# JettHuang/jet-pbrt

Hardware: AMD Instinct MI355X
Metric: Msamples/sec (whole node) + per-pixel L2 vs CPU ref, cornell_box 1024spp (higher is better)
Workload: dtype f32

## Files before the change

### jet-pbrt_amd/csrc/jp_common.h

```cpp
#pragma once
#include "jp_shading.h"

using namespace jp;

extern __shared__ float4 s_dyn[];

#define JP_SHADE_CLASSES 6

struct DevCounters
{
	unsigned int n_queue[2];
	unsigned int n_shadow;
	unsigned int pad;
	unsigned long long closest, closest_hit, shadow, shadow_occ;
	unsigned long long cert_fallback;
};

struct Queues
{
	float4 *ray_o[2], *ray_d[2], *beta[2];
	float2 *hit;
	float4 *lacc;
	float4 *sh_o;
	float4 *sh_d, *sh_c;
	unsigned int *blk_q[2], *blk_sh;
	unsigned int cap;
	unsigned int R;
};

struct RenderConst
{
	int width, height, spp, max_depth;
	unsigned int seed;
	int band_rows, shard_index, shard_count;
	int npix;
	int local_rows;
	int s0, sbatch;
	int n_planes;
	int tiled;
	int compact;
	int slot_bits;
	int sampler_debug;
	int class_mask;
	int lane_index, lane_count, lane_rows;
};

__device__ __forceinline__ float rngf(const RenderConst& rc, uint32_t key, uint32_t dim) { return rc.sampler_debug ? 0.5f : jp_rng_float(key, dim); }

#define FLAG_BOUNCE(f) ((f) & 0xff)
#define FLAG_SPEC(f)   (((f) >> 8) & 1)
#define FLAG_DIM(f)    (((unsigned)(f)) >> 16)
#define MK_FLAGS(bounce, spec, dim) (((bounce) & 0xff) | ((spec) ? 0x100 : 0) | ((int)(dim) << 16))

__device__ __forceinline__ void pixel_of(const RenderConst& rc, int pix, int& x, int& y)
{
	int lx, r;
	if (rc.tiled)
	{
		const int t = pix >> 6, i = pix & 63, tpr = rc.width >> 4;
		const int ty = t / tpr, tx = t - ty * tpr;
		lx = (tx << 4) + (i & 15); r = (ty << 2) + (i >> 4);
	}
	else { r = pix / rc.width; lx = pix - r * rc.width; }
	x = lx;
	if (rc.lane_count > 1) { const int m = r / rc.lane_rows; r = (rc.lane_index + m * rc.lane_count) * rc.lane_rows + (r - m * rc.lane_rows); }
	const int j = r / rc.band_rows;
	y = (rc.shard_index + j * rc.shard_count) * rc.band_rows + (r - j * rc.band_rows);
}

__device__ __forceinline__ unsigned int wave_take(unsigned int* ctr, unsigned int n)
{
	unsigned int v = 0;
	if ((threadIdx.x & 63) == 0) v = atomicAdd(ctr, n);
	return (unsigned int)__builtin_amdgcn_readfirstlane((int)v);
}


#define JP_TEX_IMAGE_TAG 0x80000000u
#define JP_TEX_COLOR_TAG 0x40000000u
struct TexView
{
	const int4* desc;
	const float4* col;
	const unsigned int* texels;
	const int* mat_tex;
	const float2* prim_uv;
	unsigned int* side;
};
```

### jet-pbrt_amd/csrc/jp_kernels.hip

```cpp
#include "jp_common.h"
#include "jp_tex.h"
#include "jp_xbsdf.h"

#include <cstdio>
#include <cstring>
#include <string>
#include <vector>
#include <algorithm>
#include <cmath>
#include <mutex>
#include <thread>
#include "jp_lbvh.h"
#include "jp_ploc.h"

__global__ void __launch_bounds__(JP_BLOCK) k_raygen(SceneView sc, Queues q, RenderConst rc, DevCounters* cnt)
{
	const unsigned int total = (unsigned int)rc.npix * rc.sbatch;
	const unsigned int nchunks = (total + JP_BLOCK - 1) / JP_BLOCK;
	const unsigned int G = gridDim.x, b = blockIdx.x;
	if (b == 0 && threadIdx.x == 0) { cnt->n_queue[0] = total; cnt->n_queue[1] = 0; cnt->n_shadow = 0; }
	unsigned int filled = 0;
	const unsigned int K = (nchunks + G - 1) / G, npb = (unsigned int)rc.npix / JP_BLOCK;
	for (unsigned int k = 0, j0 = 0; k < K; k++, j0 += JP_BLOCK)
	{
// ... 51 lines not shown
template <> struct SceneAccess<1>
{
	float4 *nodes, *prims; int* stack; int depth;
	__device__ __forceinline__ SceneAccess(const SceneView& sc, int depth_) : depth(depth_)
	{
		stack = (int*)s_dyn + threadIdx.x;
		nodes = s_dyn + (depth * JP_BLOCK) / 4;
		prims = nodes + 5 * sc.n_nodes;
		for (int i = threadIdx.x; i < 4 * sc.n_nodes; i += JP_BLOCK) nodes[5 * (i >> 2) + (i & 3)] = sc.nodes[i];
		for (int i = threadIdx.x; i < 4 * sc.n_prims; i += JP_BLOCK) prims[5 * (i >> 2) + (i & 3)] = sc.prims[i];
		__syncthreads();
	}
	template <bool kAnyHit> __device__ __forceinline__ int trace(const SceneView&, V3 o, V3 d, float tmin, float& tmax) const
	{ return traverse<kAnyHit, 5>(nodes, prims, o, d, tmin, tmax, stack); }
};
template <> struct SceneAccess<2>
{
	float4* prims;
	__device__ __forceinline__ SceneAccess(const SceneView& sc, int)
	{
		prims = s_dyn;
		for (int i = threadIdx.x; i < 4 * sc.n_prims; i += JP_BLOCK) prims[5 * (i >> 2) + (i & 3)] = sc.prims[i];
		__syncthreads();
	}
	template <bool kAnyHit> __device__ __forceinline__ int trace(const SceneView& sc, V3 o, V3 d, float tmin, float& tmax) const
	{ return traverse_flat<kAnyHit, 5>(sc.flat, sc.n_flat, sc.n_prims, prims, o, d, tmin, tmax); }
};

template <> struct SceneAccess<3>
{
	const float4* prims; unsigned int* stack;
	__device__ __forceinline__ SceneAccess(const SceneView& sc, int) : prims(sc.prims), stack((unsigned int*)s_dyn + threadIdx.x) {}
	template <bool kAnyHit> __device__ __forceinline__ int trace(const SceneView& sc, V3 o, V3 d, float tmin, float& tmax) const
	{ return traverse_wide<kAnyHit>(sc.wide, prims, o, d, tmin, tmax, stack); }
};

template <> struct SceneAccess<4>
{
	WalkStack stack;
	__device__ __forceinline__ SceneAccess(const SceneView&, int depth) { stack.lds = (int*)s_dyn + threadIdx.x; stack.spill = nullptr; stack.cap = depth - 1; stack.stride = 0; }
	template <bool kAnyHit> __device__ __forceinline__ int trace(const SceneView& sc, V3 o, V3 d, float tmin, float& tmax) const
	{ return walk_ray<4, kAnyHit>(sc, o, d, tmin, tmax, stack); }
};

template <> struct SceneAccess<6>
{
	WalkStack stack;
	__device__ __forceinline__ SceneAccess(const SceneView&, int depth) { stack.lds = (int*)s_dyn + threadIdx.x; stack.spill = nullptr; stack.cap = depth - 1; stack.stride = 0; }
	template <bool kAnyHit> __device__ __forceinline__ int trace(const SceneView& sc, V3 o, V3 d, float tmin, float& tmax) const
	{ return walk_ray<6, kAnyHit>(sc, o, d, tmin, tmax, stack); }
};

template <> struct SceneAccess<5>
{
	const float4 *nodes, *prims; int* stack;
	__device__ __forceinline__ SceneAccess(const SceneView& sc, int) : nodes(sc.nodes), prims(sc.prims), stack((int*)s_dyn + threadIdx.x) {}
	template <bool kAnyHit> __device__ __forceinline__ int trace(const SceneView&, V3 o, V3 d, float tmin, float& tmax) const
	{ return traverse_ref<kAnyHit>(nodes, prims, o, d, tmin, tmax, stack); }
};

template <int kMode>
__global__ void __launch_bounds__(JP_BLOCK) k_extend(SceneView sc, Queues q, int cur, int depth, DevCounters* cnt)
{
	SceneAccess<kMode> acc(sc, depth);
	const unsigned int b = blockIdx.x, n = q.blk_q[cur][b], rbase = b * q.R;
	if (b == 0 && threadIdx.x == 0) { cnt->closest += cnt->n_queue[cur]; cnt->n_queue[cur ^ 1] = 0; cnt->n_shadow = 0; }
	unsigned int h = 0;
	float4 ro = make_float4(0, 0, 0, 0), rd = make_float4(0, 0, 1, 0);
	if (threadIdx.x < n) { ro = q.ray_o[cur][rbase + threadIdx.x]; rd = q.ray_d[cur][rbase + threadIdx.x]; }
	for (unsigned int j = threadIdx.x; j < n; j += JP_BLOCK)
	{
		const unsigned int i = rbase + j;
		const float4 co = ro, cd = rd;
		if (j + JP_BLOCK < n) { ro = q.ray_o[cur][i + JP_BLOCK]; rd = q.ray_d[cur][i + JP_BLOCK]; }
		float tmax = JP_INF;
		const int hit = acc.template trace<false>(sc, xyz(co), xyz(cd), 0.001f, tmax);
		q.hit[i] = make_float2(tmax, __int_as_float(hit));
		h += hit >= 0 ? 1u : 0u;
	}
	for (int off = 32; off > 0; off >>= 1) h += __shfl_down(h, off);
	if ((threadIdx.x & 63) == 0 && h) atomicAdd(&cnt->closest_hit, (unsigned long long)h);
}

#ifndef JP_SHADE_TILE
#define JP_SHADE_TILE 8192
#endif
template <bool kTab, bool kPrims, bool kStage, bool kSort, bool kTex>
__device__ __forceinline__ void shade_body(SceneView sc, Queues q, RenderConst rc, int cur, DevCounters* cnt, const TexView& tv)
{
	static_assert(kTab || !kPrims, "k_shade: primitive records in LDS only together with the tables");
	constexpr int kWaves = JP_BLOCK / 64, kMaxSeg = (JP_SHADE_TILE / JP_BLOCK) * kWaves;
	static_assert(JP_SHADE_TILE % JP_BLOCK == 0 && JP_SHADE_TILE <= 65536, "k_shade: tile positions are 16-bit");
	__shared__ unsigned short s_idx[kSort ? JP_SHADE_TILE : 1];
	__shared__ unsigned char s_key[kSort ? JP_SHADE_TILE : 1];
	__shared__ unsigned int s_cnt[kSort ? JP_SHADE_CLASSES * kMaxSeg : 1];
	__shared__ unsigned int s_wsum[kWaves];
	__shared__ unsigned int s_ctr[3];
	const unsigned int lane = threadIdx.x & 63u;
	const int n_tab = 2 * sc.n_lights + 4 * sc.n_mats + (sc.n_mats + 3) / 4, n_tab_all = n_tab + (kPrims ? 8 * sc.n_prims : 0);
	float4* s_lights = s_dyn;
	float4* s_mats = s_lights + 2 * sc.n_lights;
	int* s_mtype = (int*)(s_mats + 4 * sc.n_mats);
	float4* s_prims = s_dyn + n_tab;
	int4* s_meta = (int4*)(s_prims + 4 * sc.n_prims);
	const float4* s_frames = s_prims + 5 * sc.n_prims;
	float4* s_stage = s_dyn + n_tab_all + threadIdx.x;
	const unsigned int b = blockIdx.x, n = q.blk_q[cur][b];
	const int nxt = cur ^ 1;
#ifdef JP_SHADE_TIMING
	unsigned long long t_acc[10] = { 0, 0, 0, 0, 0, 0, 0, 0, 0, 0 }, t_last = __builtin_amdgcn_s_memtime();
#endif
	if (kTab)
	{
		for (int i = threadIdx.x; i < n_tab_all; i += 2 * JP_BLOCK)
		{
			const bool two = i + JP_BLOCK < n_tab_all;
			const float4 a = sc.shade_tab[i], c2 = two ? sc.shade_tab[i + JP_BLOCK] : a;
			s_dyn[i] = a; if (two) s_dyn[i + JP_BLOCK] = c2;
		}
	}
	if (n == 0) { if (threadIdx.x == 0) { q.blk_q[nxt][b] = 0; q.blk_sh[b] = 0; } return; }
	if (threadIdx.x == 0) { s_ctr[0] = 0; s_ctr[1] = 0; s_ctr[2] = 0; }
	__syncthreads();
	const float4* lights = kTab ? (const float4*)s_lights : sc.lights;
	const float4* mats = kTab ? (const float4*)s_mats : sc.mats;
	const int* mat_type = kTab ? (const int*)s_mtype : sc.mat_type;
	const float4* prims = kPrims ? (const float4*)s_prims : sc.prims;
	const int4* meta_t = kPrims ? (const int4*)s_meta : sc.meta;
	const unsigned int rbase = b * q.R;
	const unsigned int t0 = 0, count = n;
	JP_TS(0);
	if (kSort)
	{
		constexpr unsigned int seg = kMaxSeg, nctr = JP_SHADE_CLASSES * kMaxSeg;
		const unsigned int tid = threadIdx.x;
		const unsigned int plane = tid & 63u, wave = tid >> 6, npass = (count + JP_BLOCK - 1) / JP_BLOCK;
		const unsigned long long ltm = (1ull << plane) - 1ull;
		#pragma unroll 1
		for (unsigned int r0 = 0; r0 < npass; r0 += 8)
		{
			int pi[8];
			#pragma unroll
			for (int u = 0; u < 8; u++)
			{
				const unsigned int j = (r0 + u) * JP_BLOCK + tid;
				pi[u] = j < count ? __float_as_int(q.hit[rbase + t0 + j].y) : -2;
			}
			#pragma unroll
			for (int u = 0; u < 8; u++)
			{
				const unsigned int r = r0 + u;
				if (r >= npass) break;
				unsigned int key = JP_SHADE_CLASSES;
				if (pi[u] != -2)
				{
					int m = -1; if (pi[u] >= 0) m = meta_t[pi[u]].y;
					key = m >= 0 ? 1u + (unsigned int)mat_type[m] : 0u;
				}
				s_key[r * JP_BLOCK + tid] = (unsigned char)key;
				unsigned int mine = 0;
				#pragma unroll
				for (int c = 0; c < JP_SHADE_CLASSES; c++)
				{
					unsigned int nc = 0;
					if ((rc.class_mask >> c) & 1) nc = (unsigned int)__popcll(__ballot(key == (unsigned int)c));
					if (plane == (unsigned int)c) mine = nc;
				}
				if (plane < JP_SHADE_CLASSES) s_cnt[plane * seg + r * kWaves + wave] = mine;
			}
		}
		__syncthreads();
		{
			static_assert(JP_SHADE_CLASSES * kMaxSeg <= 3 * JP_BLOCK, "k_shade: three counters per thread");
			unsigned int v[3], t = 0;
			#pragma unroll
			for (int i = 0; i < 3; i++)
			{
				const unsigned int at = 3 * tid + i;
				v[i] = (at < nctr && (at % seg) / kWaves < npass) ? s_cnt[at] : 0u; t += v[i];
			}
			unsigned int incl = t;
			#pragma unroll
			for (int off = 1; off < 64; off <<= 1) { const unsigned int o = __shfl_up(incl, off); if (plane >= (unsigned int)off) incl += o; }
			if (plane == 63) s_wsum[wave] = incl;
			__syncthreads();
			unsigned int base = incl - t;
			#pragma unroll
			for (int w = 0; w < kWaves; w++) if ((unsigned int)w < wave) base += s_wsum[w];
			#pragma unroll
// ... 174 lines not shown
		JP_TS(5);
#ifdef JP_DBG_SKIP_SAMPLE
		if (false)
#else
		if (shaded)
#endif
		{
			const float ux = rngf(rc, key, dim), uy = rngf(rc, key, dim + 1); dim += 2;
			BsdfSample bs = sample_local(c, wo, ux, uy);
			bs.wi = to_world(fr, bs.wi);
			if (!(isblack(bs.f) || bs.pdf == 0.f))
			{
				nspec = (bs.flags & BS_SPECULAR) != 0;
				if (bounce >= 3)
				{
					const float qq = smax(0.05f, 1 - maxcomp(bs.f));
					const float ur = rngf(rc, key, dim++);
					if (!(ur < qq))
					{
						nbeta = cmul(beta, bs.f * absdot(bs.wi, N) / (bs.pdf * (1 - qq)));
						alive = true;
					}
				}
				else
				{
					nbeta = cmul(beta, bs.f * absdot(bs.wi, N) / bs.pdf);
					alive = true;
				}
				nd = bs.wi; nbounce = bounce + 1;
			}
		}
		JP_TS(6);
		unsigned int j = 0;
		const unsigned long long lt = (1ull << lane) - 1ull;
		const unsigned long long ma = __ballot(alive);
		if (kStage)
		{
			const unsigned long long ms = __ballot(k > 0);
			if (ma | ms)
			{
				const unsigned int base = wave_take(&s_ctr[1], (unsigned int)__popcll(ma) | ((unsigned int)__popcll(ms) << 16));
				j = rbase + (base & 0xffffu) + (unsigned int)__popcll(ma & lt);
				qs = rbase + (base >> 16) + (unsigned int)__popcll(ms & lt);
			}
			if (k > 0)
			{
				q.sh_o[qs] = make_float4(p.x, p.y, p.z, __int_as_float(slot | (k << rc.slot_bits)));
				for (int kk = 0; kk < k; kk++)
				{
					q.sh_d[(size_t)kk * q.cap + qs] = s_stage[(2 * kk) * JP_BLOCK];
					q.sh_c[(size_t)kk * q.cap + qs] = s_stage[(2 * kk + 1) * JP_BLOCK];
				}
			}
		}
		else if (ma) j = rbase + wave_take(&s_ctr[1], (unsigned int)__popcll(ma)) + (unsigned int)__popcll(ma & lt);
		if (alive)
		{
			q.ray_o[nxt][j] = make_float4(p.x, p.y, p.z, __int_as_float(slot));
			q.ray_d[nxt][j] = make_float4(nd.x, nd.y, nd.z, __int_as_float(MK_FLAGS(nbounce, nspec, dim)));
			q.beta[nxt][j] = make_float4(nbeta.x, nbeta.y, nbeta.z, __int_as_float((int)key));
		}
		JP_TS(7);
#ifdef JP_SHADE_TIMING
		asm volatile("s_waitcnt vmcnt(0)" ::: "memory");
		JP_TS(9);
#endif
	}
	JP_TS(2);
	__syncthreads();
	JP_TS(8);
#ifdef JP_SHADE_TIMING
	if (lane == 0) for (int i = 0; i < 10; i++) atomicAdd(&g_shade_t[i], t_acc[i]);
	if (lane == 0) atomicAdd(&g_shade_t[15], 1ull);
#endif
	if (threadIdx.x == 0)
	{
		const unsigned int run_q = kStage ? (s_ctr[1] & 0xffffu) : s_ctr[1], run_sh = kStage ? (s_ctr[1] >> 16) : s_ctr[2];
		q.blk_q[nxt][b] = run_q; q.blk_sh[b] = run_sh;
		if (run_q) atomicAdd(&cnt->n_queue[nxt], run_q);
		if (run_sh) atomicAdd(&cnt->n_shadow, run_sh);
	}
}
template <bool kTab, bool kPrims, bool kStage, bool kSort>
__global__ void __launch_bounds__(JP_BLOCK) k_shade(SceneView sc, Queues q, RenderConst rc, int cur, DevCounters* cnt)
{
	const TexView tv = {};
	shade_body<kTab, kPrims, kStage, kSort, false>(sc, q, rc, cur, cnt, tv);
}

template <int kMode>
__global__ void __launch_bounds__(JP_BLOCK, 4) k_shadow(SceneView sc, Queues q, RenderConst rc, int depth, DevCounters* cnt)
{
#ifdef JP_TRAV_TIMING
	unsigned long long t_acc[10] = { 0, 0, 0, 0, 0, 0, 0, 0, 0, 0 }, t_last = __builtin_amdgcn_s_memtime();
#endif
	SceneAccess<kMode> acc(sc, depth);
	const unsigned int b = blockIdx.x, E = q.blk_sh[b], rbase = b * q.R;
	JP_TT(0);
	unsigned int rays = 0, occ = 0;
	float4 so_n = make_float4(0, 0, 0, 0), sd_n = make_float4(0, 0, 1, 0);
	if (threadIdx.x < E) { so_n = q.sh_o[rbase + threadIdx.x]; sd_n = q.sh_d[rbase + threadIdx.x]; }
	for (unsigned int j = threadIdx.x; j < E; j += JP_BLOCK)
	{
		const unsigned int e = rbase + j;
#ifdef JP_TRAV_TIMING
		JP_TT(1);
		asm volatile("s_waitcnt vmcnt(0)" ::: "memory");
		JP_TT(2);
#endif
		const float4 so = so_n; float4 sd = sd_n;
		if (j + JP_BLOCK < E) { so_n = q.sh_o[e + JP_BLOCK]; sd_n = q.sh_d[e + JP_BLOCK]; }
		const int packed = __float_as_int(so.w);
		const int slot = packed & ((1 << rc.slot_bits) - 1), n = (int)((unsigned int)packed >> rc.slot_bits);
		if (n == 0) continue;
		bool any = false;
		const float4 L = q.lacc[slot];
		V3 a = mk(L.x, L.y, L.z);
		for (int k = 0; k < n; k++)
		{
			const float4 c4 = q.sh_c[(size_t)k * q.cap + e];
			float tmax = sd.w;
			const V3 dir = xyz(sd);
			if (k + 1 < n) sd = q.sh_d[(size_t)(k + 1) * q.cap + e];
			JP_TT(3);
#ifdef JP_TRAV_TIMING
			int hit;
			if constexpr (kMode == 2)
			{
				const unsigned int m = flat_boxes<false>(sc.flat, sc.n_flat, xyz(so), dir, 0.001f, tmax);
				JP_TT(4);
				hit = flat_prims<true, false, 5>(m, acc.prims, xyz(so), dir, 0.001f, tmax);
				JP_TT(5);
			}
			else hit = acc.template trace<true>(sc, xyz(so), dir, 0.001f, tmax);
#else
			const int hit = acc.template trace<true>(sc, xyz(so), dir, 0.001f, tmax);
#endif
			rays++;
			if (hit >= 0) occ++;
			else { a = a + xyz(c4); any = true; }
			JP_TT(6);
		}
		if (any) q.lacc[slot] = make_float4(a.x, a.y, a.z, 0.f);
		JP_TT(7);
	}
#ifdef JP_TRAV_TIMING
	JP_TT(1);
	if ((threadIdx.x & 63) == 0) { for (int i = 0; i < 8; i++) atomicAdd(&g_shade_t[i], t_acc[i]); atomicAdd(&g_shade_t[15], 1ull); }
#endif
	for (int off = 32; off > 0; off >>= 1) { rays += __shfl_down(rays, off); occ += __shfl_down(occ, off); }
	if ((threadIdx.x & 63) == 0) { if (rays) atomicAdd(&cnt->shadow, (unsigned long long)rays); if (occ) atomicAdd(&cnt->shadow_occ, (unsigned long long)occ); }
}

template <int kMode, bool kAnyHit, bool kVote>
__device__ __forceinline__ void persist_turn(Walker<kMode>& w, const SceneView& sc, const WalkStack& stack, bool pool)
{
	const int nh = __popcll(__ballot(!w.done && w.heavy())), nl = __popcll(__ballot(!w.done && !w.heavy()));
	const bool heavyTurn = kVote ? nh > nl : w.heavy();
	if (kVote) { JP_TURN(heavyTurn ? 3 : 0, 1); JP_TURN(heavyTurn ? 4 : 1, heavyTurn ? nh : nl); JP_TURN(heavyTurn ? 5 : 2, nh + nl); if (!pool) { JP_TURN(8, 1); JP_TURN(9, nh + nl); JP_TURN(10, heavyTurn ? nh : nl); } }
	if (!w.done && (w.heavy() == heavyTurn)) w.template step<kAnyHit>(sc, stack);
}
__device__ __forceinline__ unsigned int lane_rank(unsigned long long m) { return __builtin_amdgcn_mbcnt_hi((unsigned int)(m >> 32), __builtin_amdgcn_mbcnt_lo((unsigned int)m, 0u)); }

#ifndef JP_CERT_WAVES
#define JP_CERT_WAVES 8
#endif
template <int kMode, int kRefill, bool kVote>
// ... 451 lines not shown
```

### jet-pbrt_amd/csrc/jp_shading.h

```cpp
#pragma once
#include "jp_device.h"
#define JP_HD_INLINE __host__ __device__ __forceinline__

namespace jp
{
__device__ __forceinline__ void sincos_d(float xf, double* s, double* c)
{
	const double x = (double)xf;
	const double kd = rint(x * 0.63661977236758134308);
	const int k = (int)kd;
	double r = fma(-kd, 1.57079632679489655800e+00, x);
	r = fma(-kd, 6.12323399573676603587e-17, r);
	const double r2 = r * r;
	double sp = fma(r2, -7.6471637318198164759e-13, 1.6059043836821614599e-10);
	sp = fma(sp, r2, -2.5052108385441718775e-08);
	sp = fma(sp, r2, 2.7557319223985890653e-06);
	sp = fma(sp, r2, -1.9841269841269841270e-04);
	sp = fma(sp, r2, 8.3333333333333333333e-03);
	sp = fma(sp, r2, -1.6666666666666666667e-01);
	sp = fma(sp * r2, r, r);
	double cp = fma(r2, 4.7794773323873852974e-14, -1.1470745597729724714e-11);
	cp = fma(cp, r2, 2.0876756987868098979e-09);
	cp = fma(cp, r2, -2.7557319223985890653e-07);
	cp = fma(cp, r2, 2.4801587301587301587e-05);
	cp = fma(cp, r2, -1.3888888888888888889e-03);
	cp = fma(cp, r2, 4.1666666666666666667e-02);
	cp = fma(cp, r2, -0.5);
	cp = fma(cp, r2, 1.0);
	const double ss = (k & 1) ? cp : sp, cc = (k & 1) ? sp : cp;
	*s = (k & 2) ? -ss : ss;
	*c = ((k + 1) & 2) ? -cc : cc;
}

__device__ __constant__ int g_sincosf_mode = 0;

template <bool kFma>
JP_HD_INLINE void sincosf_libm(float y, float* sp, float* cp)
{
	union { float f; unsigned int u; } bits; bits.f = y;
	const unsigned int top = (bits.u >> 20) & 0x7ffu;
	const double x = (double)y;
	double xs, x2; int n = 0;
	if (top <= 0x3f3u)
	{
		if (top <= 0x397u) { *sp = y; *cp = 1.0f; return; }
		xs = x; x2 = x * x;
	}
	else
	{
		const double r = x * 0x1.45f306dc9c883p+23;
		n = ((int)r + 0x800000) >> 24;
		const double xr = kFma ? fma(-(double)n, 0x1.921fb54442d18p+0, x) : x - (double)n * 0x1.921fb54442d18p+0;
		const double sgn = ((n & 3) == 1 || (n & 3) == 2) ? -1.0 : 1.0;
		xs = xr * sgn; x2 = xr * xr;
	}
	const double t = (n & 2) ? -1.0 : 1.0;
	const double c0 = t, c1 = t * -0x1.ffffffd0c621cp-2, c2 = t * 0x1.55553e1068f19p-5, c3 = t * -0x1.6c087e89a359dp-10, c4 = t * 0x1.99343027bf8c3p-16;
	const double s1 = -0x1.555545995a603p-3, s2 = 0x1.1107605230bc4p-7, s3 = -0x1.994eb3774cf24p-13;
	const double x3 = x2 * xs, x4 = x2 * x2;
	const double x5 = x2 * x3, x6 = x2 * x4;
	double c1v, as, ac, bs, bc, S, C;
	if (kFma)
	{
		c1v = fma(x2, c1, c0); as = fma(x2, s3, s2); ac = fma(x2, c4, c3);
		bs = fma(x3, s1, xs); bc = fma(x4, c2, c1v);
		S = fma(as, x5, bs); C = fma(ac, x6, bc);
	}
	else
	{
		c1v = c0 + x2 * c1; as = s2 + x2 * s3; ac = c3 + x2 * c4;
		bs = xs + x3 * s1; bc = c1v + x4 * c2;
		S = bs + x5 * as; C = bc + x6 * ac;
	}
	const float fs = (float)S, fc = (float)C;
	if (n & 1) { *sp = fc; *cp = fs; } else { *sp = fs; *cp = fc; }
}

__device__ __forceinline__ void sincos_f(float xf, float* s, float* c)
{
	const int mode = g_sincosf_mode;
	if (mode == 1 && fabsf(xf) < 120.f) sincosf_libm<true>(xf, s, c);
	else if (mode == 2 && fabsf(xf) < 120.f) sincosf_libm<false>(xf, s, c);
	else { double sd, cd; sincos_d(xf, &sd, &cd); *s = (float)sd; *c = (float)cd; }
}

#define JP_2PI      (2.0f * JP_PI)
#define JP_PI_OVER2 (JP_PI / 2.0f)
#define JP_PI_OVER4 (JP_PI / 4.0f)
#define JP_INV_PI   (1.0f / JP_PI)

enum { BS_REFLECTION = 1, BS_TRANSMISSION = 2, BS_SPECULAR = 4, BS_DIFFUSE = 8, BS_GLOSSY = 16 };
enum { CL_LAMBERT = 0, CL_MIRROR = 1, CL_FRESNEL_SPECULAR = 2, CL_MICROFACET = 3 };
enum { FR_CONDUCTOR = 0, FR_DIELECTRIC = 1 };

struct Frame { V3 s, t, n; };
__device__ __forceinline__ Frame frame_from_z(V3 nn)
{
	Frame f; f.n = normalize(nn);
	V3 tmp = (fabsf(f.n.x) > 0.99f) ? mk(0, 1, 0) : mk(1, 0, 0);
	f.t = normalize(cross(f.n, tmp));
	f.s = normalize(cross(f.t, f.n));
	return f;
}
__device__ __forceinline__ V3 to_local(const Frame& f, V3 w) { return mk(dot(f.s, w), dot(f.t, w), dot(f.n, w)); }
__device__ __forceinline__ V3 to_world(const Frame& f, V3 l) { return f.s * l.x + f.t * l.y + f.n * l.z; }

struct Closure
{
	int kind;
	V3 c0, c1;
	float eta_t;
	float ax, ay;
	int fresnel; V3 feta, fk;
	float lam_o;
};
__device__ __forceinline__ bool is_delta(const Closure& c) { return c.kind == CL_MIRROR || c.kind == CL_FRESNEL_SPECULAR; }

struct BsdfSample { V3 f, wi; float pdf; int flags; };

__device__ __forceinline__ void concentric_disk(float ux, float uy, float& px, float& py)
{
	ux = ux * 2.f - 1.f; uy = uy * 2.f - 1.f;
	if (ux == 0 && uy == 0) { px = 0; py = 0; }
	else
	{
		float radius, theta;
		if (fabsf(ux) > fabsf(uy)) { radius = ux; theta = JP_PI_OVER4 * (uy / ux); }
		else { radius = uy; theta = JP_PI_OVER2 - JP_PI_OVER4 * (ux / uy); }
		float st, ct; sincos_f(theta, &st, &ct);
		px = ct * radius; py = st * radius;
	}
}
__device__ __forceinline__ V3 cosine_hemisphere(float ux, float uy)
{
	float px, py; concentric_disk(ux, uy, px, py);
	float z = sqrtf(smax(0.f, 1 - px * px - py * py));
	return mk(px, py, z);
}
__device__ __forceinline__ V3 uniform_sphere(float ux, float uy)
{
	float z = 1 - 2 * ux;
// ... 340 lines not shown
```

### jet-pbrt_amd/csrc/jp_upload.h

```cpp
#pragma once
namespace
{
struct HV3 { float x, y, z; };
inline HV3 hsub(HV3 a, HV3 b) { HV3 r = { a.x - b.x, a.y - b.y, a.z - b.z }; return r; }
inline HV3 hcross(HV3 a, HV3 v) { HV3 r = { a.y * v.z - a.z * v.y, a.z * v.x - a.x * v.z, a.x * v.y - a.y * v.x }; return r; }
inline float hlen(HV3 a) { return std::sqrt(a.x * a.x + a.y * a.y + a.z * a.z); }
inline HV3 hld(const float* p) { HV3 r = { p[0], p[1], p[2] }; return r; }

struct ItemTree { std::vector<int> left, right; std::vector<float> bounds; int height = 0; };
int item_tree_build(const std::vector<float>& ib, std::vector<int>& idx, int start, int end, ItemTree& t, int depth)
{
	const int node = (int)t.left.size(); t.left.push_back(0); t.right.push_back(0); t.bounds.resize(t.bounds.size() + 6);
	t.height = std::max(t.height, depth);
	float nb[6] = { 1e30f, 1e30f, 1e30f, -1e30f, -1e30f, -1e30f }, cb[6] = { 1e30f, 1e30f, 1e30f, -1e30f, -1e30f, -1e30f };
	for (int i = start; i < end; i++)
	{
		const float* b = &ib[6 * (size_t)idx[i]];
		for (int a = 0; a < 3; a++) { nb[a] = std::min(nb[a], b[a]); nb[3 + a] = std::max(nb[3 + a], b[3 + a]); const float c = 0.5f * (b[a] + b[3 + a]); cb[a] = std::min(cb[a], c); cb[3 + a] = std::max(cb[3 + a], c); }
	}
	std::memcpy(&t.bounds[6 * (size_t)node], nb, sizeof(nb));
	if (end - start == 1) { t.left[node] = -idx[start] - 1; return node; }
	auto area = [](const float* b) { const float dx = b[3] - b[0], dy = b[4] - b[1], dz = b[5] - b[2]; return (dx < 0 || dy < 0 || dz < 0) ? 0.f : dx * dy + dy * dz + dz * dx; };
	const int NB = 16; float bestCost = 3.0e38f; int bestAxis = -1, bestBin = -1;
	for (int a = 0; a < 3; a++)
// ... 528 lines not shown
		if (ty == JP_LIGHT_AREA)
		{
			int p = s->light_prim[i]; dp = devPrimOf[p];
			int t = s->prim_shape_type[p], k = s->prim_shape_index[p]; float area;
			if (t == JP_SHAPE_TRIANGLE) area = 0.5f * hlen(hcross(hsub(hld(s->tri_p1 + 3 * k), hld(s->tri_p0 + 3 * k)), hsub(hld(s->tri_p2 + 3 * k), hld(s->tri_p0 + 3 * k))));
			else if (t == JP_SHAPE_RECTANGLE) area = hlen(hcross(hsub(hld(s->rect_p0 + 3 * k), hld(s->rect_p1 + 3 * k)), hsub(hld(s->rect_p2 + 3 * k), hld(s->rect_p1 + 3 * k))));
			else if (t == JP_SHAPE_DISK) { const float kPi = (float)3.14159265358979323846; area = kPi * s->disk_radius[k] * s->disk_radius[k]; }
			else { const float kPi = (float)3.14159265358979323846; float r2 = s->sph_radius[k] * s->sph_radius[k]; area = 4 * kPi * r2; }
			inv_area = 1 / area;
		}
		else if (ty == JP_LIGHT_ENVIRONMENT) { nenv++; envsum[0] += rad[0]; envsum[1] += rad[1]; envsum[2] += rad[2]; }
		float df; std::memcpy(&df, &dp, 4);
		lights[2 * i + 1] = make_float4(df, inv_area, 0, 0);
		if (ty == JP_LIGHT_POINT || ty == JP_LIGHT_DIRECTION) lights[2 * i + 1] = make_float4(s->light_vec[3 * i], s->light_vec[3 * i + 1], s->light_vec[3 * i + 2], 0);
	}

	auto up = [&](void** dst, const void* src, size_t bytes) -> hipError_t {
		hipError_t e = hipMalloc(dst, std::max<size_t>(bytes, 16)); if (e != hipSuccess) return e;
		return hipMemcpy(*dst, src, bytes, hipMemcpyHostToDevice);
	};
	if (!device_build)
	{
		HIP_TRY(up(&c->d_nodes, nodes.data(), nodes.size() * sizeof(float4)));
		HIP_TRY(up(&c->d_prims, prims.data(), prims.size() * sizeof(float4)));
		HIP_TRY(up(&c->d_meta, meta.data(), meta.size() * sizeof(int4)));
	}
	HIP_TRY(up(&c->d_mats, mats.data(), mats.size() * sizeof(float4)));
	HIP_TRY(up(&c->d_mat_type, mtype.data(), mtype.size() * sizeof(int)));
	HIP_TRY(up(&c->d_lights, lights.data(), lights.size() * sizeof(float4)));
	{
		std::vector<float4> tabv;
		tabv.insert(tabv.end(), lights.begin(), lights.begin() + 2 * (size_t)s->n_lights);
		tabv.insert(tabv.end(), mats.begin(), mats.begin() + 4 * (size_t)s->n_materials);
		const size_t at = tabv.size(); tabv.resize(at + ((size_t)s->n_materials + 3) / 4, make_float4(0, 0, 0, 0));
		if (s->n_materials > 0) std::memcpy(&tabv[at], mtype.data(), (size_t)s->n_materials * sizeof(int));
		if (!device_build)
		{
			tabv.insert(tabv.end(), prims.begin(), prims.end());
			const size_t am = tabv.size(); tabv.resize(am + meta.size());
			std::memcpy(&tabv[am], meta.data(), meta.size() * sizeof(int4));
			auto hnorm = [](HV3 a) { const float l = hlen(a); HV3 r = { a.x / l, a.y / l, a.z / l }; return r; };
			for (size_t pi = 0; pi < meta.size(); pi++)
			{
				const float4 g3 = prims[4 * pi + 3], g1 = prims[4 * pi + 1];
				int type; std::memcpy(&type, &g3.w, 4);
				const HV3 nn = type == JP_SHAPE_DISK ? HV3{ g1.x, g1.y, g1.z } : HV3{ g3.x, g3.y, g3.z };
				const HV3 n = hnorm(nn);
				const HV3 tmp = std::fabs(n.x) > 0.99f ? HV3{ 0, 1, 0 } : HV3{ 1, 0, 0 };
				const HV3 t = hnorm(hcross(n, tmp)), sv = hnorm(hcross(t, n));
				tabv.push_back(make_float4(n.x, n.y, n.z, 0)); tabv.push_back(make_float4(sv.x, sv.y, sv.z, 0)); tabv.push_back(make_float4(t.x, t.y, t.z, 0));
			}
		}
		HIP_TRY(up(&c->d_shade_tab, tabv.data(), tabv.size() * sizeof(float4)));
	}
	if (use_wide && !dev_wide) HIP_TRY(up(&c->d_wide, wide.data(), wide.size() * sizeof(uint32_t)));
	if ((use_q4 && !dev_q4) || use_cert) HIP_TRY(up(&c->d_q4, q4.data(), q4.size() * sizeof(uint32_t)));
	if (use_cert) HIP_TRY(up(&c->d_refbox, refbox.data(), refbox.size() * sizeof(float4)));
	if (!flat.empty()) HIP_TRY(up(&c->d_flat, flat.data(), flat.size() * sizeof(float4)));

	ScenePlan& p = c->plan; SceneView& v = p.sv;
	v.nodes = (const float4*)c->d_nodes; v.n_nodes = (int)(n4nodes / 4);
	v.prims = (const float4*)c->d_prims; v.meta = (const int4*)c->d_meta; v.n_prims = (int)nmeta;
	v.mats = (const float4*)c->d_mats; v.mat_type = (const int*)c->d_mat_type; v.n_mats = s->n_materials;
	v.lights = (const float4*)c->d_lights; v.n_lights = s->n_lights; v.shade_tab = (const float4*)c->d_shade_tab;
	v.env_sum = make_float3(envsum[0], envsum[1], envsum[2]); v.n_env = nenv;
	v.world_radius = s->world_radius; v.cam = s->camera;
	v.flat = (const float4*)c->d_flat; v.n_flat = (int)(flat.size() / 2);
	v.wide = (const uint4*)c->d_wide; v.n_wide = dev_wide ? dev_n_wide : (int)(wide.size() / 20);
	v.q4 = (const uint4*)c->d_q4; v.n_q4 = dev_q4 ? dev_n_q4 : (int)(q4.size() / 16);
	v.refbox = (const float4*)c->d_refbox; v.cert_pad = cert_pad; v.cert_pad_eye = cert_pad_eye; p.cert = use_cert;
	p.use_q4 = use_q4; p.q4_shadow = use_q4 && opt_flag(op.q4_shadow, true);
	p.stack_depth = std::max(2, height + 2);
	p.stack_depth_q4 = (use_q4 || use_cert) ? 3 * q4_height + 2 : 0;
	size_t scene_bytes = (n4nodes + n4prims) / 4 * 5 * sizeof(float4);
	size_t prim_bytes = n4prims / 4 * 5 * sizeof(float4);
	size_t stack_bytes = (size_t)p.stack_depth * JP_BLOCK * sizeof(int);
	p.scene_in_lds = !device_build && scene_bytes + stack_bytes <= 40 * 1024;
	p.trav_mode = use_wide ? 3 : ((!flat.empty() && prim_bytes <= 40 * 1024) ? 2 : (p.scene_in_lds ? 1 : 0));
	if (!use_wide && op.traversal > 0) { const int m = op.traversal - 1; if (m == 0 || (m == 1 && p.scene_in_lds)) p.trav_mode = m; }
	if (use_wide) p.scene_in_lds = false;
	if (ref_sem) p.trav_mode = 5;
	p.lds_bytes = p.trav_mode == 2 ? prim_bytes : (p.trav_mode == 1 ? stack_bytes + scene_bytes : stack_bytes);
	p.lds_bytes_shadow = p.trav_mode == 3 ? (size_t)2 * (wide_height + 2) * JP_BLOCK * sizeof(int) : p.lds_bytes;
	{
		size_t tab = ((size_t)2 * s->n_lights + (size_t)4 * s->n_materials) * sizeof(float4) + (size_t)s->n_materials * sizeof(int) + 16;
		p.tables_in_lds = tab <= 16 * 1024;
		const size_t shade_static = (size_t)JP_SHADE_TILE * 3 + (size_t)JP_SHADE_CLASSES * (JP_SHADE_TILE / JP_BLOCK) * (JP_BLOCK / 64) * 4 + 128;
		const size_t prim_part = n4prims * sizeof(float4) + nmeta * sizeof(int4) + 3 * nmeta * sizeof(float4);
		p.shade_prims_in_lds = p.tables_in_lds && p.scene_in_lds && tab + prim_part <= 24 * 1024;
		p.shade_lds_bytes = p.tables_in_lds ? tab + (p.shade_prims_in_lds ? prim_part : 0) : 0;
		const size_t stage_bytes = 16 + (size_t)std::max(1, planes) * 2 * JP_BLOCK * sizeof(float4);
		p.stage_nee = p.tables_in_lds && std::max(1, planes) <= 4 && shade_static + p.shade_lds_bytes + stage_bytes <= 64 * 1024;
		if (p.stage_nee) p.shade_lds_bytes += stage_bytes;
	}
	p.n_planes = std::max(1, planes);
	{
		bool kinds[8] = { false, false, false, false, false, false, false, false }; int nk = 0;
		for (int i = 0; i < s->n_primitives; i++) { const int m = s->prim_material[i]; const int k = m < 0 ? 7 : s->mat_type[m]; if (!kinds[k]) { kinds[k] = true; nk++; } }
		p.stack_lds_words = op.stack_lds_words >= 2 ? (op.stack_lds_words & ~1) : 12;
		p.persist = ((p.trav_mode == 0 || p.trav_mode == 3 || p.trav_mode == 5) && s->n_primitives > 1024) ? 16 : 0;
		if (op.persist != 0) p.persist = op.persist < 0 ? 0 : op.persist;
		p.vote = opt_flag(op.vote, p.trav_mode != 5 || p.cert);
		p.class_mask = 1; for (int k = 0; k < 5; k++) if (kinds[k]) p.class_mask |= 2 << k;
		p.shade_sort = opt_flag(op.shade_sort, nk > 1);
	}
	p.has_null_material = hasNull; c->cert_fell_back = false;
	p.have_scene = true;
	return JP_OK;
}


extern "C" int jp_upload_scene_textured(JpContext* c, const JpScene* s, const JpTextures* t)
{
	if (!c || !s) return fail(JP_ERR_INVALID_ARGUMENT, "jp_upload_scene_textured: null argument");
	if (!t) return jp_upload_scene(c, s);
	if (t->struct_bytes < (int32_t)sizeof(JpTextures)) return fail(JP_ERR_INVALID_ARGUMENT, "jp_upload_scene_textured: JpTextures.struct_bytes smaller than this library's JpTextures");
	if (t->n_textures < 0 || t->n_textures > (1 << 28)) return fail(JP_ERR_INVALID_ARGUMENT, "jp_upload_scene_textured: n_textures out of range");
	if (t->n_textures == 0) return jp_upload_scene(c, s);
	const int nt = t->n_textures;
	if (!t->tex_type || !t->tex_color) return fail(JP_ERR_INVALID_ARGUMENT, "jp_upload_scene_textured: null tex_type / tex_color");
	if (t->n_materials != s->n_materials) return fail(JP_ERR_INVALID_ARGUMENT, "jp_upload_scene_textured: n_materials differs from the scene's");
	if (t->n_triangles != s->n_triangles) return fail(JP_ERR_INVALID_ARGUMENT, "jp_upload_scene_textured: n_triangles differs from the scene's");
	if (t->n_materials > 0 && (!t->mat_texture || !s->mat_type)) return fail(JP_ERR_INVALID_ARGUMENT, "jp_upload_scene_textured: null mat_texture");
	long long pool = 0;
	for (int i = 0; i < nt; i++)
	{
		const int ty = t->tex_type[i];
		if (ty < JP_TEXTURE_SOLID || ty > JP_TEXTURE_IMAGE) return fail(JP_ERR_INVALID_ARGUMENT, "jp_upload_scene_textured: unknown texture type");
		if (ty == JP_TEXTURE_IMAGE)
		{
			if (!t->tex_width || !t->tex_height || !t->tex_offset || !t->texels) return fail(JP_ERR_INVALID_ARGUMENT, "jp_upload_scene_textured: image texture without tex_width / tex_height / tex_offset / texels");
			const long long w = t->tex_width[i], h = t->tex_height[i], off = t->tex_offset[i];
			if (w < 1 || w > 16384 || h < 1 || h > 16384) return fail(JP_ERR_INVALID_ARGUMENT, "jp_upload_scene_textured: image size out of range (1 .. 16384 per side)");
			if (off < 0 || t->n_texel_bytes < 0 || off > t->n_texel_bytes - 3 * w * h) return fail(JP_ERR_INVALID_ARGUMENT, "jp_upload_scene_textured: image texels beyond n_texel_bytes");
			pool += w * h;
		}
		else
		{
			const int nc = ty == JP_TEXTURE_CHECKER ? 6 : 3;
			for (int k = 0; k < nc; k++) if (!std::isfinite(t->tex_color[6 * (size_t)i + k])) return fail(JP_ERR_INVALID_ARGUMENT, "jp_upload_scene_textured: colour not finite");
		}
	}
	if (pool > 0x7fffffffll) return fail(JP_ERR_INVALID_ARGUMENT, "jp_upload_scene_textured: more than 2^31 texels in all");
	int ntm = 0;
	for (int m = 0; m < t->n_materials; m++)
	{
		const int k = t->mat_texture[m];
		if (k < -1 || k >= nt) return fail(JP_ERR_INVALID_ARGUMENT, "jp_upload_scene_textured: mat_texture out of range");
		if (k < 0) continue;
		const int mt = s->mat_type[m];
		if (mt != JP_MAT_MATTE && mt != JP_MAT_MIRROR && mt != JP_MAT_PLASTIC) return fail(JP_ERR_INVALID_ARGUMENT, "jp_upload_scene_textured: a texture on a glass or metal material (its [0..2] is eta, not a colour)");
		ntm++;
	}
	if (s->n_primitives > 0 && (!s->prim_shape_type || !s->prim_shape_index)) return fail(JP_ERR_INVALID_ARGUMENT, "jp_upload_scene_textured: null array");
	const int st = jp_upload_scene(c, s);
	if (st != JP_OK) return st;
	if (ntm == 0) return JP_OK;

	std::vector<int4> desc(nt); std::vector<float4> col(2 * (size_t)nt); std::vector<unsigned int> texels((size_t)pool);
	size_t at = 0;
	for (int i = 0; i < nt; i++)
	{
		const float* cc = t->tex_color + 6 * (size_t)i;
		desc[i] = make_int4(t->tex_type[i], 0, 0, 0);
		col[2 * i] = make_float4(0, 0, 0, 0); col[2 * i + 1] = make_float4(0, 0, 0, 0);
		if (t->tex_type[i] == JP_TEXTURE_IMAGE)
		{
			const int w = t->tex_width[i], h = t->tex_height[i];
			desc[i].y = w; desc[i].z = h; desc[i].w = (int)at;
			const uint8_t* src = t->texels + t->tex_offset[i];
			for (size_t k = 0; k < (size_t)w * h; k++) texels[at + k] = (unsigned int)src[3 * k] | ((unsigned int)src[3 * k + 1] << 8) | ((unsigned int)src[3 * k + 2] << 16) | 0xff000000u;
			at += (size_t)w * h;
		}
		else
		{
			col[2 * i] = make_float4(cc[0], cc[1], cc[2], 0);
			if (t->tex_type[i] == JP_TEXTURE_CHECKER) col[2 * i + 1] = make_float4(cc[3], cc[4], cc[5], 0);
		}
	}
	std::vector<int> mt(t->mat_texture, t->mat_texture + t->n_materials);
	std::vector<float2> puv(3 * (size_t)s->n_primitives, make_float2(0, 0));
	if (t->tri_uv)
		for (int p = 0; p < s->n_primitives; p++)
			if (s->prim_shape_type[p] == JP_SHAPE_TRIANGLE)
			{
				const float* u = t->tri_uv + 6 * (size_t)s->prim_shape_index[p];
				for (int k = 0; k < 3; k++) puv[3 * (size_t)p + k] = make_float2(u[2 * k], u[2 * k + 1]);
// ... 20 lines not shown
```

Before: 2969.

## Alias shade sort scratch with NEE staging in dynamic LDS and raise occupancy

Moves the shade kernel's sort keys and per-class counters from static shared memory into the dynamic LDS region, where they overlap the NEE staging buffer. The host budgets the dynamic region as the larger of the two instead of their sum. This shrinks the shade kernel's LDS footprint so more blocks can be resident, and __launch_bounds__(JP_BLOCK,4) asks the compiler to fit four blocks per CU. The double-precision constants in the sincos routines are pinned in scalar registers through an empty asm, to cut the VGPRs used for literal materialisation. Risks: register spills under the new bound, and corruption if the sort scratch and the staging buffer are ever live at the same time.

```diff
diff --git a/jet-pbrt_amd/csrc/jp_common.h b/jet-pbrt_amd/csrc/jp_common.h
--- a/jet-pbrt_amd/csrc/jp_common.h
+++ b/jet-pbrt_amd/csrc/jp_common.h
@@ -5,7 +5,7 @@
 
 extern __shared__ float4 s_dyn[];
 
-#define JP_SHADE_CLASSES 6
+#include "jp_shade_lds.h"
 
 struct DevCounters
 {
diff --git a/jet-pbrt_amd/csrc/jp_kernels.hip b/jet-pbrt_amd/csrc/jp_kernels.hip
--- a/jet-pbrt_amd/csrc/jp_kernels.hip
+++ b/jet-pbrt_amd/csrc/jp_kernels.hip
@@ -157,9 +157,6 @@
 	if ((threadIdx.x & 63) == 0 && h) atomicAdd(&cnt->closest_hit, (unsigned long long)h);
 }
 
-#ifndef JP_SHADE_TILE
-#define JP_SHADE_TILE 8192
-#endif
 template <bool kTab, bool kPrims, bool kStage, bool kSort, bool kTex>
 __device__ __forceinline__ void shade_body(SceneView sc, Queues q, RenderConst rc, int cur, DevCounters* cnt, const TexView& tv)
 {
@@ -167,19 +164,22 @@
 	constexpr int kWaves = JP_BLOCK / 64, kMaxSeg = (JP_SHADE_TILE / JP_BLOCK) * kWaves;
 	static_assert(JP_SHADE_TILE % JP_BLOCK == 0 && JP_SHADE_TILE <= 65536, "k_shade: tile positions are 16-bit");
 	__shared__ unsigned short s_idx[kSort ? JP_SHADE_TILE : 1];
-	__shared__ unsigned char s_key[kSort ? JP_SHADE_TILE : 1];
-	__shared__ unsigned int s_cnt[kSort ? JP_SHADE_CLASSES * kMaxSeg : 1];
 	__shared__ unsigned int s_wsum[kWaves];
 	__shared__ unsigned int s_ctr[3];
 	const unsigned int lane = threadIdx.x & 63u;
-	const int n_tab = 2 * sc.n_lights + 4 * sc.n_mats + (sc.n_mats + 3) / 4, n_tab_all = n_tab + (kPrims ? 8 * sc.n_prims : 0);
+	const int n_tab = JP_SHADE_TAB_F4(sc.n_lights, sc.n_mats), n_tab_all = n_tab + (kPrims ? JP_SHADE_PRIM_F4 * sc.n_prims : 0);
 	float4* s_lights = s_dyn;
 	float4* s_mats = s_lights + 2 * sc.n_lights;
 	int* s_mtype = (int*)(s_mats + 4 * sc.n_mats);
 	float4* s_prims = s_dyn + n_tab;
 	int4* s_meta = (int4*)(s_prims + 4 * sc.n_prims);
 	const float4* s_frames = s_prims + 5 * sc.n_prims;
-	float4* s_stage = s_dyn + n_tab_all + threadIdx.x;
+	float4* s_scr = s_dyn + (kTab ? n_tab_all : 0);
+	float4* s_stage = s_scr + threadIdx.x;
+	static_assert(JP_SHADE_KEY_BYTES == JP_SHADE_TILE * sizeof(unsigned char) && JP_SHADE_KEY_BYTES % sizeof(float4) == 0, "k_shade: the keys end on a 16-byte boundary");
+	static_assert(JP_SHADE_CNT_BYTES == JP_SHADE_CLASSES * kMaxSeg * sizeof(unsigned int), "k_shade: one counter per (class, pass, wave), as jp_shade_lds.h budgets them");
+	unsigned char* s_key = (unsigned char*)s_scr;
+	unsigned int* s_cnt = (unsigned int*)(s_scr + JP_SHADE_KEY_BYTES / sizeof(float4));
 	const unsigned int b = blockIdx.x, n = q.blk_q[cur][b];
 	const int nxt = cur ^ 1;
 #ifdef JP_SHADE_TIMING
@@ -520,7 +520,7 @@
 	}
 }
 template <bool kTab, bool kPrims, bool kStage, bool kSort>
-__global__ void __launch_bounds__(JP_BLOCK) k_shade(SceneView sc, Queues q, RenderConst rc, int cur, DevCounters* cnt)
+__global__ void __launch_bounds__(JP_BLOCK, 4) k_shade(SceneView sc, Queues q, RenderConst rc, int cur, DevCounters* cnt)
 {
 	const TexView tv = {};
 	shade_body<kTab, kPrims, kStage, kSort, false>(sc, q, rc, cur, cnt, tv);
diff --git a/jet-pbrt_amd/csrc/jp_shade_lds.h b/jet-pbrt_amd/csrc/jp_shade_lds.h
--- /dev/null
+++ b/jet-pbrt_amd/csrc/jp_shade_lds.h
@@ -0,0 +1,50 @@
+#pragma once
+#include <stddef.h>
+
+#ifndef JP_BLOCK
+#define JP_BLOCK 256
+#endif
+#ifndef JP_SHADE_TILE
+#define JP_SHADE_TILE 8192
+#endif
+#define JP_SHADE_CLASSES 6
+#define JP_SHADE_KEY_BYTES  (JP_SHADE_TILE)
+#define JP_SHADE_CNT_BYTES  (JP_SHADE_CLASSES * (JP_SHADE_TILE / JP_BLOCK) * (JP_BLOCK / 64) * 4)
+#define JP_SHADE_SORT_BYTES (JP_SHADE_KEY_BYTES + JP_SHADE_CNT_BYTES)
+#define JP_SHADE_TAB_F4(n_lights, n_mats) (2 * (n_lights) + 4 * (n_mats) + ((n_mats) + 3) / 4)
+#define JP_SHADE_PRIM_F4 8
+
+struct JpShadeLds
+{
+	bool tables_in_lds, prims_in_lds, stage_nee;
+	size_t tab_bytes;
+	size_t prim_bytes;
+	size_t key_bytes;
+	size_t sort_bytes;
+	size_t stage_bytes;
+	size_t static_bytes;
+	size_t dynamic_bytes;
+	size_t total_bytes;
+};
+
+static inline JpShadeLds jp_shade_lds_layout(int n_lights, int n_mats, size_t n_prims, bool scene_in_lds, int n_planes, bool sort)
+{
+	JpShadeLds L;
+	const size_t f4 = 16;
+	const size_t tab = ((size_t)2 * n_lights + (size_t)4 * n_mats) * f4 + (size_t)n_mats * 4 + 16;
+	const size_t prim_part = n_prims * JP_SHADE_PRIM_F4 * f4;
+	L.tables_in_lds = tab <= 16 * 1024;
+	L.prims_in_lds = L.tables_in_lds && scene_in_lds && tab + prim_part <= 24 * 1024;
+	L.tab_bytes = L.tables_in_lds ? tab : 0;
+	L.prim_bytes = L.prims_in_lds ? prim_part : 0;
+	L.key_bytes = sort ? (size_t)JP_SHADE_KEY_BYTES : 0;
+	L.sort_bytes = sort ? (size_t)JP_SHADE_SORT_BYTES : 0;
+	L.static_bytes = ((sort ? (size_t)JP_SHADE_TILE * 2 + (JP_BLOCK / 64) * 4 : 0) + 3 * 4 + 15) / 16 * 16;
+	const size_t stage = (size_t)n_planes * 2 * JP_BLOCK * f4;
+	const size_t with_stage = L.static_bytes + L.tab_bytes + L.prim_bytes + (stage > L.sort_bytes ? stage : L.sort_bytes);
+	L.stage_nee = L.tables_in_lds && n_planes <= 4 && with_stage <= 64 * 1024;
+	L.stage_bytes = L.stage_nee ? stage : 0;
+	L.dynamic_bytes = L.tab_bytes + L.prim_bytes + (L.stage_bytes > L.sort_bytes ? L.stage_bytes : L.sort_bytes);
+	L.total_bytes = L.static_bytes + L.dynamic_bytes;
+	return L;
+}
diff --git a/jet-pbrt_amd/csrc/jp_shading.h b/jet-pbrt_amd/csrc/jp_shading.h
--- a/jet-pbrt_amd/csrc/jp_shading.h
+++ b/jet-pbrt_amd/csrc/jp_shading.h
@@ -4,27 +4,36 @@
 
 namespace jp
 {
+JP_HD_INLINE double jp_kd(double v)
+{
+#if defined(__HIP_DEVICE_COMPILE__)
+	asm volatile("" : "+s"(v));
+#endif
+	return v;
+}
+#define JP_KD(c) jp_kd(c)
+
 __device__ __forceinline__ void sincos_d(float xf, double* s, double* c)
 {
 	const double x = (double)xf;
-	const double kd = rint(x * 0.63661977236758134308);
+	const double kd = rint(x * JP_KD(0.63661977236758134308));
 	const int k = (int)kd;
-	double r = fma(-kd, 1.57079632679489655800e+00, x);
-	r = fma(-kd, 6.12323399573676603587e-17, r);
+	double r = fma(-kd, JP_KD(1.57079632679489655800e+00), x);
+	r = fma(-kd, JP_KD(6.12323399573676603587e-17), r);
 	const double r2 = r * r;
-	double sp = fma(r2, -7.6471637318198164759e-13, 1.6059043836821614599e-10);
-	sp = fma(sp, r2, -2.5052108385441718775e-08);
-	sp = fma(sp, r2, 2.7557319223985890653e-06);
-	sp = fma(sp, r2, -1.9841269841269841270e-04);
-	sp = fma(sp, r2, 8.3333333333333333333e-03);
-	sp = fma(sp, r2, -1.6666666666666666667e-01);
+	double sp = fma(r2, JP_KD(-7.6471637318198164759e-13), JP_KD(1.6059043836821614599e-10));
+	sp = fma(sp, r2, JP_KD(-2.5052108385441718775e-08));
+	sp = fma(sp, r2, JP_KD(2.7557319223985890653e-06));
+	sp = fma(sp, r2, JP_KD(-1.9841269841269841270e-04));
+	sp = fma(sp, r2, JP_KD(8.3333333333333333333e-03));
+	sp = fma(sp, r2, JP_KD(-1.6666666666666666667e-01));
 	sp = fma(sp * r2, r, r);
-	double cp = fma(r2, 4.7794773323873852974e-14, -1.1470745597729724714e-11);
-	cp = fma(cp, r2, 2.0876756987868098979e-09);
-	cp = fma(cp, r2, -2.7557319223985890653e-07);
-	cp = fma(cp, r2, 2.4801587301587301587e-05);
-	cp = fma(cp, r2, -1.3888888888888888889e-03);
-	cp = fma(cp, r2, 4.1666666666666666667e-02);
+	double cp = fma(r2, JP_KD(4.7794773323873852974e-14), JP_KD(-1.1470745597729724714e-11));
+	cp = fma(cp, r2, JP_KD(2.0876756987868098979e-09));
+	cp = fma(cp, r2, JP_KD(-2.7557319223985890653e-07));
+	cp = fma(cp, r2, JP_KD(2.4801587301587301587e-05));
+	cp = fma(cp, r2, JP_KD(-1.3888888888888888889e-03));
+	cp = fma(cp, r2, JP_KD(4.1666666666666666667e-02));
 	cp = fma(cp, r2, -0.5);
 	cp = fma(cp, r2, 1.0);
 	const double ss = (k & 1) ? cp : sp, cc = (k & 1) ? sp : cp;
@@ -48,15 +57,15 @@
 	}
 	else
 	{
-		const double r = x * 0x1.45f306dc9c883p+23;
+		const double r = x * JP_KD(0x1.45f306dc9c883p+23);
 		n = ((int)r + 0x800000) >> 24;
-		const double xr = kFma ? fma(-(double)n, 0x1.921fb54442d18p+0, x) : x - (double)n * 0x1.921fb54442d18p+0;
+		const double xr = kFma ? fma(-(double)n, JP_KD(0x1.921fb54442d18p+0), x) : x - (double)n * JP_KD(0x1.921fb54442d18p+0);
 		const double sgn = ((n & 3) == 1 || (n & 3) == 2) ? -1.0 : 1.0;
 		xs = xr * sgn; x2 = xr * xr;
 	}
 	const double t = (n & 2) ? -1.0 : 1.0;
-	const double c0 = t, c1 = t * -0x1.ffffffd0c621cp-2, c2 = t * 0x1.55553e1068f19p-5, c3 = t * -0x1.6c087e89a359dp-10, c4 = t * 0x1.99343027bf8c3p-16;
-	const double s1 = -0x1.555545995a603p-3, s2 = 0x1.1107605230bc4p-7, s3 = -0x1.994eb3774cf24p-13;
+	const double c0 = t, c1 = t * JP_KD(-0x1.ffffffd0c621cp-2), c2 = t * JP_KD(0x1.55553e1068f19p-5), c3 = t * JP_KD(-0x1.6c087e89a359dp-10), c4 = t * JP_KD(0x1.99343027bf8c3p-16);
+	const double s1 = JP_KD(-0x1.555545995a603p-3), s2 = JP_KD(0x1.1107605230bc4p-7), s3 = JP_KD(-0x1.994eb3774cf24p-13);
 	const double x3 = x2 * xs, x4 = x2 * x2;
 	const double x5 = x2 * x3, x6 = x2 * x4;
 	double c1v, as, ac, bs, bc, S, C;
diff --git a/jet-pbrt_amd/csrc/jp_upload.h b/jet-pbrt_amd/csrc/jp_upload.h
--- a/jet-pbrt_amd/csrc/jp_upload.h
+++ b/jet-pbrt_amd/csrc/jp_upload.h
@@ -634,27 +634,21 @@
 	if (ref_sem) p.trav_mode = 5;
 	p.lds_bytes = p.trav_mode == 2 ? prim_bytes : (p.trav_mode == 1 ? stack_bytes + scene_bytes : stack_bytes);
 	p.lds_bytes_shadow = p.trav_mode == 3 ? (size_t)2 * (wide_height + 2) * JP_BLOCK * sizeof(int) : p.lds_bytes;
-	{
-		size_t tab = ((size_t)2 * s->n_lights + (size_t)4 * s->n_materials) * sizeof(float4) + (size_t)s->n_materials * sizeof(int) + 16;
-		p.tables_in_lds = tab <= 16 * 1024;
-		const size_t shade_static = (size_t)JP_SHADE_TILE * 3 + (size_t)JP_SHADE_CLASSES * (JP_SHADE_TILE / JP_BLOCK) * (JP_BLOCK / 64) * 4 + 128;
-		const size_t prim_part = n4prims * sizeof(float4) + nmeta * sizeof(int4) + 3 * nmeta * sizeof(float4);
-		p.shade_prims_in_lds = p.tables_in_lds && p.scene_in_lds && tab + prim_part <= 24 * 1024;
-		p.shade_lds_bytes = p.tables_in_lds ? tab + (p.shade_prims_in_lds ? prim_part : 0) : 0;
-		const size_t stage_bytes = 16 + (size_t)std::max(1, planes) * 2 * JP_BLOCK * sizeof(float4);
-		p.stage_nee = p.tables_in_lds && std::max(1, planes) <= 4 && shade_static + p.shade_lds_bytes + stage_bytes <= 64 * 1024;
-		if (p.stage_nee) p.shade_lds_bytes += stage_bytes;
+	bool kinds[8] = { false, false, false, false, false, false, false, false }; int nk = 0;
+	for (int i = 0; i < s->n_primitives; i++) { const int m = s->prim_material[i]; const int k = m < 0 ? 7 : s->mat_type[m]; if (!kinds[k]) { kinds[k] = true; nk++; } }
+	p.shade_sort = opt_flag(op.shade_sort, nk > 1);
+	{
+		const JpShadeLds L = jp_shade_lds_layout(s->n_lights, s->n_materials, nmeta, p.scene_in_lds, std::max(1, planes), p.shade_sort);
+		p.tables_in_lds = L.tables_in_lds; p.shade_prims_in_lds = L.prims_in_lds; p.stage_nee = L.stage_nee;
+		p.shade_lds_bytes = L.dynamic_bytes;
 	}
 	p.n_planes = std::max(1, planes);
 	{
-		bool kinds[8] = { false, false, false, false, false, false, false, false }; int nk = 0;
-		for (int i = 0; i < s->n_primitives; i++) { const int m = s->prim_material[i]; const int k = m < 0 ? 7 : s->mat_type[m]; if (!kinds[k]) { kinds[k] = true; nk++; } }
 		p.stack_lds_words = op.stack_lds_words >= 2 ? (op.stack_lds_words & ~1) : 12;
 		p.persist = ((p.trav_mode == 0 || p.trav_mode == 3 || p.trav_mode == 5) && s->n_primitives > 1024) ? 16 : 0;
 		if (op.persist != 0) p.persist = op.persist < 0 ? 0 : op.persist;
 		p.vote = opt_flag(op.vote, p.trav_mode != 5 || p.cert);
 		p.class_mask = 1; for (int k = 0; k < 5; k++) if (kinds[k]) p.class_mask |= 2 << k;
-		p.shade_sort = opt_flag(op.shade_sort, nk > 1);
 	}
 	p.has_null_material = hasNull; c->cert_fell_back = false;
 	p.have_scene = true;
```

Result: faster. 3012 (median of 6 runs) (+1.5%).
